# foollh/PicoPose

Hardware: AMD Instinct MI355X
Metric: image-crops/sec (224x224, 162 templates) (higher is better)
Workload: dtype f32 tensors; networks: f32 operands split into 2 f16 terms (22 bits) on f16 MFMA with f32 accumulate; stage-1 contraction: f16 MFMA operands, f32 accumulate, exact f32 re-evaluation of near-ties; PnP f64

## Files before the change

### picopose_amd/csrc/pp_sample.hip

```cpp

#include <hip/hip_runtime.h>
#include <stdint.h>
#include "../../include/picopose_hip.h"
#include "pp_common.h"
#include "pp_corr_dev.h"
#include "pp_crop_dev.h"

namespace {

typedef float f4 __attribute__((ext_vector_type(4)));
typedef _Float16 h8_t __attribute__((ext_vector_type(8)));

__device__ __forceinline__ float resize_blend(float a, float b, float c, float d, float hx, float lx, float hy, float ly, float mul) {
#pragma clang fp contract(off)
    const float top = fmaf(hx, a, lx * b), bot = fmaf(hx, c, lx * d);
    return (hy * top + ly * bot) * mul;
}

__global__ __launch_bounds__(256) void resize_kernel(const float* __restrict__ in, int H, int W, int C,
                                                     int Ho, int Wo, float mul, float* __restrict__ out,
                                                     _Float16* __restrict__ out_hl, int terms) {
    const int b = blockIdx.z, oy = blockIdx.y, tid = threadIdx.x;
    const float sy = Ho > 1 ? (float)(H - 1) / (float)(Ho - 1) : 0.f;
    const float sx = Wo > 1 ? (float)(W - 1) / (float)(Wo - 1) : 0.f;
    const float fy = sy * (float)oy;
    const int y0 = (int)fy, y1 = y0 + (y0 < H - 1 ? 1 : 0);
    const float ly = fy - (float)y0, hy = 1.f - ly;
    const float* ib = in + (size_t)b * H * W * C;
    if (out_hl) {
        _Float16* oh = out_hl + ((size_t)b * Ho + oy) * Wo * terms * C;
        float* of = out ? out + ((size_t)b * Ho + oy) * Wo * C : nullptr;
        const int C8 = C >> 3;
        for (int i = blockIdx.x * 256 + tid; i < Wo * C8; i += gridDim.x * 256) {
            const int ox = i / C8, c = (i - ox * C8) * 8;
            const float fx = sx * (float)ox;
            const int x0 = (int)fx, x1 = x0 + (x0 < W - 1 ? 1 : 0);
            const float lx = fx - (float)x0, hx = 1.f - lx;
            typedef _Float16 h8 __attribute__((ext_vector_type(8)));
            h8 hh, ll;
#pragma unroll
            for (int q = 0; q < 2; ++q) {
                const int cc = c + 4 * q;
                const f4 a = *(const f4*)(ib + ((size_t)y0 * W + x0) * C + cc), bq = *(const f4*)(ib + ((size_t)y0 * W + x1) * C + cc);
                const f4 cq = *(const f4*)(ib + ((size_t)y1 * W + x0) * C + cc), dq = *(const f4*)(ib + ((size_t)y1 * W + x1) * C + cc);
// ... 11 lines not shown
            }
            *(h8*)(oh + ((size_t)ox * C + c) * terms) = hh;
            if (terms == 2) *(h8*)(oh + (size_t)ox * 2 * C + 2 * c + 8) = ll;
        }
        return;
    }
    float* ob = out + ((size_t)b * Ho + oy) * Wo * C;
    if ((C & 3) == 0 && (((uintptr_t)in | (uintptr_t)out) & 15) == 0) {
        const int C4 = C >> 2;
        for (int i = blockIdx.x * 256 + tid; i < Wo * C4; i += gridDim.x * 256) {
            const int ox = i / C4, c = (i - ox * C4) * 4;
            const float fx = sx * (float)ox;
            const int x0 = (int)fx, x1 = x0 + (x0 < W - 1 ? 1 : 0);
            const float lx = fx - (float)x0, hx = 1.f - lx;
            const f4 a = *(const f4*)(ib + ((size_t)y0 * W + x0) * C + c), bq = *(const f4*)(ib + ((size_t)y0 * W + x1) * C + c);
            const f4 cq = *(const f4*)(ib + ((size_t)y1 * W + x0) * C + c), dq = *(const f4*)(ib + ((size_t)y1 * W + x1) * C + c);
            f4 v;
#pragma unroll
            for (int k = 0; k < 4; ++k) v[k] = resize_blend(a[k], bq[k], cq[k], dq[k], hx, lx, hy, ly, mul);
            *(f4*)(ob + (size_t)ox * C + c) = v;
        }
        return;
    }
    for (int i = blockIdx.x * 256 + tid; i < Wo * C; i += gridDim.x * 256) {
        const int ox = i / C, c = i - ox * C;
        const float fx = sx * (float)ox;
        const int x0 = (int)fx, x1 = x0 + (x0 < W - 1 ? 1 : 0);
        const float lx = fx - (float)x0, hx = 1.f - lx;
        ob[i] = resize_blend(ib[((size_t)y0 * W + x0) * C + c], ib[((size_t)y0 * W + x1) * C + c], ib[((size_t)y1 * W + x0) * C + c],
                             ib[((size_t)y1 * W + x1) * C + c], hx, lx, hy, ly, mul);
    }
}

template <bool HL>
__global__ __launch_bounds__(256) void warp_kernel(const float* __restrict__ feat, int feat_batch,
                                                   const float* __restrict__ flow, int H, int W, int C, int ld_flow,
                                                   float* __restrict__ out, int ld_out, int terms) {
    const int b = blockIdx.y, p = blockIdx.x * 4 + (threadIdx.x >> 6), lane = threadIdx.x & 63;
    if (p >= H * W) return;
    const int y = p / W, x = p - y * W;
    const float* fl = flow + ((size_t)b * H * W + p) * ld_flow;
    const float ix = fminf(fmaxf(pp_roundtrip((float)x + fl[0], W), -2.f), (float)W + 1.f);
    const float iy = fminf(fmaxf(pp_roundtrip((float)y + fl[1], H), -2.f), (float)H + 1.f);
    const float x0f = floorf(ix), y0f = floorf(iy);
    const int x0 = (int)x0f, y0 = (int)y0f;
    const float wx1 = ix - x0f, wx0 = (x0f + 1.f) - ix, wy1 = iy - y0f, wy0 = (y0f + 1.f) - iy;
    const float* fb = feat + (size_t)(b % feat_batch) * H * W * C;
    float* o = HL ? nullptr : out + ((size_t)b * H * W + p) * ld_out;
    _Float16* oh = HL ? (_Float16*)out + ((size_t)b * H * W + p) * terms * ld_out : nullptr;
    const bool vx0 = x0 >= 0 && x0 < W, vx1 = x0 + 1 >= 0 && x0 + 1 < W;
    const bool vy0 = y0 >= 0 && y0 < H, vy1 = y0 + 1 >= 0 && y0 + 1 < H;
    typedef unsigned u4w __attribute__((ext_vector_type(4)));
    const unsigned m00 = 0u - (unsigned)(vy0 & vx0), m01 = 0u - (unsigned)(vy0 & vx1), m10 = 0u - (unsigned)(vy1 & vx0),
                   m11 = 0u - (unsigned)(vy1 & vx1);
    const int xa = min(max(x0, 0), W - 1), xb = min(max(x0 + 1, 0), W - 1), ya = min(max(y0, 0), H - 1), yb = min(max(y0 + 1, 0), H - 1);
    auto tap = [&](int yy, int xx, int c, unsigned m) __attribute__((always_inline)) -> f4 {
        const u4w raw = *(const u4w*)(fb + ((size_t)yy * W + xx) * C + c) & m;
        return __builtin_bit_cast(f4, raw);
    };
    for (int c = lane * 4; c < C; c += 256) {
        f4 acc = {0.f, 0.f, 0.f, 0.f};
        acc += tap(ya, xa, c, m00) * (wx0 * wy0);
        acc += tap(ya, xb, c, m01) * (wx1 * wy0);
        acc += tap(yb, xa, c, m10) * (wx0 * wy1);
        acc += tap(yb, xb, c, m11) * (wx1 * wy1);
        if (HL) {
            typedef _Float16 h4w __attribute__((ext_vector_type(4)));
            _Float16 h0, h1, h2, h3, l0, l1, l2, l3;
            pp_split_f16_chk(acc.x, h0, l0);
            pp_split_f16_chk(acc.y, h1, l1);
            pp_split_f16_chk(acc.z, h2, l2);
            pp_split_f16_chk(acc.w, h3, l3);
            if (terms == 2) {
                _Float16* q = oh + pp_hl_col(c, 0);
                *(h4w*)q = h4w{h0, h1, h2, h3};
                *(h4w*)(q + 8) = h4w{l0, l1, l2, l3};
            } else {
                *(h4w*)(oh + c) = h4w{h0, h1, h2, h3};
            }
        } else {
            *(f4*)(o + c) = acc;
        }
    }
}

__global__ __launch_bounds__(256) void avgpool2_kernel(const float* __restrict__ in, int H, int W, int C,
                                                       float* __restrict__ out) {
    const int Ho = H / 2, Wo = W / 2, b = blockIdx.y;
    const size_t n = (size_t)Ho * Wo * C;
    const float* ib = in + (size_t)b * H * W * C;
    float* ob = out + (size_t)b * n;
    for (size_t i = (size_t)blockIdx.x * 256 + threadIdx.x; i < n; i += (size_t)gridDim.x * 256) {
        const int c = (int)(i % C);
        const size_t q = i / C;
        const int ox = (int)(q % Wo), oy = (int)(q / Wo);
        const float* p = ib + ((size_t)(2 * oy) * W + 2 * ox) * C + c;
        ob[i] = ((p[0] + p[C]) + (p[(size_t)W * C] + p[(size_t)W * C + C])) * 0.25f;
    }
}

__global__ __launch_bounds__(256) void avgpool2_hl_kernel(const float* __restrict__ in, int H, int W, int C, float* __restrict__ out,
                                                          _Float16* __restrict__ out_hl) {
    const int Ho = H / 2, Wo = W / 2, b = blockIdx.y, C4 = C >> 2;
    const size_t n4 = (size_t)Ho * Wo * C4;
    const float* ib = in + (size_t)b * H * W * C;
    for (size_t i = (size_t)blockIdx.x * 256 + threadIdx.x; i < n4; i += (size_t)gridDim.x * 256) {
        const int c = (int)(i % C4) * 4;
        const size_t q = i / C4;
        const int ox = (int)(q % Wo), oy = (int)(q / Wo);
        const float* p = ib + ((size_t)(2 * oy) * W + 2 * ox) * C + c;
        const f4 p0 = *(const f4*)p, p1 = *(const f4*)(p + C), p2 = *(const f4*)(p + (size_t)W * C), p3 = *(const f4*)(p + (size_t)W * C + C);
        f4 v;
#pragma unroll
        for (int k = 0; k < 4; ++k) v[k] = ((p0[k] + p1[k]) + (p2[k] + p3[k])) * 0.25f;
        const size_t row = (size_t)b * Ho * Wo + q;
        if (out) *(f4*)(out + row * C + c) = v;
// ... 206 lines not shown
            const int c = i / (np >> 2), q = i - c * (np >> 2);
            *(f4*)&t[c][4 * q] = *(const f4*)(src + (size_t)c * HW + p0 + 4 * q);
        }
    } else {
        for (int i = tid; i < 3 * np; i += 256) {
            const int c = i / np, q = i - c * np;
            t[c][q] = src[(size_t)c * HW + p0 + q];
        }
    }
    __syncthreads();
    h8_t* o = (h8_t*)(out + ((size_t)j * HW + p0) * 8 * terms);
    const _Float16 z = (_Float16)0.f;
    for (int i = tid; i < np * terms; i += 256) {
        const int q = terms == 2 ? i >> 1 : i;
        _Float16 h0, l0, h1, l1, h2, l2;
        if (terms == 1 || (i & 1) == 0) {
            pp_split_f16_chk(t[0][q], h0, l0);
            pp_split_f16_chk(t[1][q], h1, l1);
            pp_split_f16_chk(t[2][q], h2, l2);
            o[i] = h8_t{h0, h1, h2, z, z, z, z, z};
        } else {
            pp_split_f16(t[0][q], h0, l0);
            pp_split_f16(t[1][q], h1, l1);
            pp_split_f16(t[2][q], h2, l2);
            o[i] = h8_t{l0, l1, l2, z, z, z, z, z};
        }
    }
}

}

PP_SAT_SETTER(pp_sat_set_sample)

extern "C" {

int pp_resize_bilinear_nhwc(const float* in, int B, int H, int W, int C, int Ho, int Wo, float mul, float* out,
                            void* stream) {
    if (!in || !out || B <= 0 || H <= 0 || W <= 0 || C <= 0 || Ho <= 0 || Wo <= 0) return PP_EINVAL;
    const bool vec = (C & 3) == 0 && (((uintptr_t)in | (uintptr_t)out) & 15) == 0;
    const int work = vec ? Wo * (C / 4) : Wo * C;
    const int gx = (work + 1023) / 1024;
    hipLaunchKernelGGL(resize_kernel, dim3(gx < 64 ? gx : 64, Ho, B), dim3(256), 0, (hipStream_t)stream, in, H, W,
                       C, Ho, Wo, mul, out, (_Float16*)nullptr, 2);
    return pp_last_launch();
}

int pp_resize_bilinear_nhwc_t(const float* in, int B, int H, int W, int C, int Ho, int Wo, float mul, void* out_hl,
                              int terms, void* stream) {
    if (!in || !out_hl || B <= 0 || H <= 0 || W <= 0 || C <= 0 || C % 8 != 0 || Ho <= 0 || Wo <= 0 ||
        (((uintptr_t)in | (uintptr_t)out_hl) & 15) != 0 || (terms != 1 && terms != 2))
        return PP_EINVAL;
    const int gx = (Wo * (C / 8) + 1023) / 1024;
    hipLaunchKernelGGL(resize_kernel, dim3(gx < 64 ? gx : 64, Ho, B), dim3(256), 0, (hipStream_t)stream, in, H, W,
                       C, Ho, Wo, mul, (float*)nullptr, (_Float16*)out_hl, terms);
    return pp_last_launch();
}

int pp_resize_bilinear_nhwc_dual(const float* in, int B, int H, int W, int C, int Ho, int Wo, float mul, float* out, void* out_hl,
                                 int terms, void* stream) {
    if (!in || !out || !out_hl || B <= 0 || H <= 0 || W <= 0 || C <= 0 || C % 8 != 0 || Ho <= 0 || Wo <= 0 ||
        (((uintptr_t)in | (uintptr_t)out | (uintptr_t)out_hl) & 15) != 0 || (terms != 1 && terms != 2))
        return PP_EINVAL;
    const int gx = (Wo * (C / 8) + 1023) / 1024;
    hipLaunchKernelGGL(resize_kernel, dim3(gx < 64 ? gx : 64, Ho, B), dim3(256), 0, (hipStream_t)stream, in, H, W,
                       C, Ho, Wo, mul, out, (_Float16*)out_hl, terms);
    return pp_last_launch();
}

int pp_resize_bilinear_nhwc_hl(const float* in, int B, int H, int W, int C, int Ho, int Wo, float mul, void* out_hl,
                               void* stream) {
    return pp_resize_bilinear_nhwc_t(in, B, H, W, C, Ho, Wo, mul, out_hl, 2, stream);
}

int pp_warp_nhwc(const float* feat, int feat_batch, const float* flow, int B, int H, int W, int C, int ld_flow,
                 float* out, int ld_out, void* stream) {
    if (!feat || !flow || !out || B <= 0 || H <= 0 || W <= 0 || C <= 0 || C % 4 != 0 || ld_flow < 2 || feat_batch <= 0 ||
        ld_out < C || ld_out % 4 != 0 || ((uintptr_t)out % 16) != 0)
        return PP_EINVAL;
    hipLaunchKernelGGL(warp_kernel<false>, dim3((H * W + 3) / 4, B), dim3(256), 0, (hipStream_t)stream, feat, feat_batch, flow,
                       H, W, C, ld_flow, out, ld_out, 2);
    return pp_last_launch();
}

int pp_warp_nhwc_t(const float* feat, int feat_batch, const float* flow, int B, int H, int W, int C, int ld_flow,
                   void* out_hl, int ld_h, int terms, void* stream) {
    if (!feat || !flow || !out_hl || B <= 0 || H <= 0 || W <= 0 || C <= 0 || C % 8 != 0 || ld_flow < 2 || feat_batch <= 0 ||
        ld_h < C || ld_h % 8 != 0 || ((uintptr_t)out_hl % 16) != 0 || (terms != 1 && terms != 2))
        return PP_EINVAL;
    hipLaunchKernelGGL(warp_kernel<true>, dim3((H * W + 3) / 4, B), dim3(256), 0, (hipStream_t)stream, feat, feat_batch, flow,
                       H, W, C, ld_flow, (float*)out_hl, ld_h, terms);
    return pp_last_launch();
}

int pp_warp_nhwc_hl(const float* feat, int feat_batch, const float* flow, int B, int H, int W, int C, int ld_flow,
                    void* out_hl, int ld_h, void* stream) {
    return pp_warp_nhwc_t(feat, feat_batch, flow, B, H, W, C, ld_flow, out_hl, ld_h, 2, stream);
}

int pp_avgpool2_nhwc(const float* in, int B, int H, int W, int C, float* out, void* stream) {
    if (!in || !out || B <= 0 || H < 2 || W < 2 || C <= 0 || H % 2 != 0 || W % 2 != 0) return PP_EINVAL;
    const size_t n = (size_t)(H / 2) * (W / 2) * C;
    const int gx = (int)((n + 255) / 256 < 1024 ? (n + 255) / 256 : 1024);
    hipLaunchKernelGGL(avgpool2_kernel, dim3(gx, B), dim3(256), 0, (hipStream_t)stream, in, H, W, C, out);
    return pp_last_launch();
}

int pp_avgpool2_hl(const float* in, int B, int H, int W, int C, float* out, void* out_hl, void* stream) {
    if (!in || !out_hl || B <= 0 || H < 2 || W < 2 || C <= 0 || H % 2 != 0 || W % 2 != 0 || C % 8 != 0) return PP_EINVAL;
    if (((uintptr_t)in | (uintptr_t)out | (uintptr_t)out_hl) % 16 != 0) return PP_EINVAL;
    const size_t n = (size_t)(H / 2) * (W / 2) * (C / 4);
    const int gx = (int)((n + 255) / 256 < 1024 ? (n + 255) / 256 : 1024);
    hipLaunchKernelGGL(avgpool2_hl_kernel, dim3(gx, B), dim3(256), 0, (hipStream_t)stream, in, H, W, C, out, (_Float16*)out_hl);
    return pp_last_launch();
}

int pp_conv_narrow_f32(const float* x, int ld_x, int B, int H, int W, int C, const float* weight, const float* bias, int ksize,
                       int n_out, const float* residual, float* out, void* stream) {
    if (!x || !weight || !out || B <= 0 || H <= 0 || C <= 0 || C % 32 != 0 || ld_x < C || ld_x % 4 != 0) return PP_EINVAL;
    if ((W != 16 && W != 32 && W != 64) || H % (256 / W) != 0 || (ksize != 1 && ksize != 3) || (n_out != 1 && n_out != 2)) return PP_EINVAL;
    if (((uintptr_t)x % 16) != 0) return PP_EINVAL;
    const int TH = 256 / W, R = ksize / 2;
    const size_t lds = (size_t)(TH + 2 * R) * (W + 2 * R) * NRW_PITCH;
    const dim3 grid((unsigned)(B * (H / TH)));
// ... 103 lines not shown
```

### picopose_amd/csrc/pp_winograd.hip

```cpp
#include <hip/hip_runtime.h>
#include <stdint.h>
#include "../../include/picopose_hip.h"
#include "pp_common.h"

namespace {

typedef float f4 __attribute__((ext_vector_type(4)));

__device__ __forceinline__ void wino_bt_d_b(const f4 (&d)[4][4], f4 (&u)[4][4]) {
    f4 t[4][4];
#pragma unroll
    for (int c = 0; c < 4; ++c) {
        t[0][c] = d[0][c] - d[2][c];
        t[1][c] = d[1][c] + d[2][c];
        t[2][c] = d[2][c] - d[1][c];
        t[3][c] = d[1][c] - d[3][c];
    }
#pragma unroll
    for (int a = 0; a < 4; ++a) {
        u[a][0] = t[a][0] - t[a][2];
        u[a][1] = t[a][1] + t[a][2];
        u[a][2] = t[a][2] - t[a][1];
        u[a][3] = t[a][1] - t[a][3];
    }
}

__global__ __launch_bounds__(256) void wino_input_kernel(const float* __restrict__ x, int ld_x, long long bstride, int B, int H, int W, int C,
                                                         int relu, float* __restrict__ U) {
    const int c4n = C >> 2;
    const long long P = (long long)B * (H >> 1) * (W >> 1), total = P * c4n;
    for (long long i = (long long)blockIdx.x * 256 + threadIdx.x; i < total; i += (long long)gridDim.x * 256) {
        const long long p = i / c4n;
        const int c = (int)(i - p * c4n) * 4;
        const int tw = W >> 1, th = H >> 1;
        const int b = (int)(p / ((long long)th * tw)), r = (int)(p - (long long)b * th * tw), ty = r / tw, tx = r - ty * tw;
        const int y0 = 2 * ty - 1, x0 = 2 * tx - 1;
// ... 122 lines not shown

__device__ __forceinline__ long long wino_logical_block() {
    const unsigned per = gridDim.x >> 3;
    return (long long)(blockIdx.x & 7) * per + (blockIdx.x >> 3);
}

#define PP_W4_BT(d0, d1, d2, d3, d4, d5, t0, t1, t2, t3, t4, t5)          \
    {                                                                     \
        const f4 a_ = d4 - 4.f * d2, b_ = d3 - 4.f * d1;                  \
        const f4 c_ = d4 - d2, e_ = 2.f * (d3 - d1);                      \
        t0 = 4.f * d0 - 5.f * d2 + d4;                                    \
        t1 = a_ + b_;                                                     \
        t2 = a_ - b_;                                                     \
        t3 = c_ + e_;                                                     \
        t4 = c_ - e_;                                                     \
        t5 = 4.f * d1 - 5.f * d3 + d5;                                    \
    }

__device__ __forceinline__ void wino_split4(f4 v, hf4& hi, hf4& lo, float& top) {
    top = fmaxf(fmaxf(top, fabsf(v[0])), fabsf(v[1]));
    top = fmaxf(fmaxf(top, fabsf(v[2])), fabsf(v[3]));
#pragma unroll
    for (int e = 0; e < 4; ++e) {
        const _Float16 h = (_Float16)v[e];
        hi[e] = h;
        lo[e] = (_Float16)(v[e] - (float)h);
    }
}

__device__ __forceinline__ void wino_note_sat(bool clamp, unsigned* sat) {
    if (sat && __builtin_amdgcn_ballot_w64(clamp) != 0ull && (threadIdx.x & 63) == 0) atomicOr(sat, 1u);
}

typedef unsigned int wu4 __attribute__((ext_vector_type(4)));
__device__ __forceinline__ unsigned wino_swap(unsigned v) { return (unsigned)__builtin_amdgcn_mov_dpp((int)v, 0xB1, 0xF, 0xF, true); }
__device__ __forceinline__ float wino_h2f(unsigned w, int hi16) { return (float)__builtin_bit_cast(_Float16, (unsigned short)(hi16 ? w >> 16 : w & 0xFFFFu)); }

__device__ __forceinline__ f4 wino_pair_unpack(wu4 q, int par) {
    const unsigned k0 = par ? q[2] : q[0], k1 = par ? q[3] : q[1];
    const unsigned r0 = wino_swap(par ? q[0] : q[2]), r1 = wino_swap(par ? q[1] : q[3]);
    return f4{wino_h2f(k0, 0) + wino_h2f(r0, 0), wino_h2f(k0, 1) + wino_h2f(r0, 1), wino_h2f(k1, 0) + wino_h2f(r1, 0), wino_h2f(k1, 1) + wino_h2f(r1, 1)};
}

__device__ __forceinline__ wu4 wino_pair_pack(int par, hf4 hi, hf4 lo) {
    const unsigned H0 = __builtin_bit_cast(unsigned, __builtin_shufflevector(hi, hi, 0, 1)), H1 = __builtin_bit_cast(unsigned, __builtin_shufflevector(hi, hi, 2, 3));
    const unsigned L0 = __builtin_bit_cast(unsigned, __builtin_shufflevector(lo, lo, 0, 1)), L1 = __builtin_bit_cast(unsigned, __builtin_shufflevector(lo, lo, 2, 3));
    const unsigned r0 = wino_swap(par ? H0 : L0), r1 = wino_swap(par ? H1 : L1);
    return wu4{par ? r0 : H0, par ? r1 : H1, par ? L0 : r0, par ? L1 : r1};
}

__device__ __forceinline__ __amdgpu_buffer_rsrc_t wino_block_rsrc(const void* base, int xi, unsigned long long block_bytes) {
    return __builtin_amdgcn_make_buffer_rsrc((void*)((const char*)base + (unsigned long long)xi * block_bytes), 0, (int)(unsigned)block_bytes, 0x00020000);
}

__device__ __forceinline__ void wino_pair_store(_Float16* grp, int par, hf4 hi, hf4 lo) {
    const unsigned H0 = __builtin_bit_cast(unsigned, __builtin_shufflevector(hi, hi, 0, 1)), H1 = __builtin_bit_cast(unsigned, __builtin_shufflevector(hi, hi, 2, 3));
    const unsigned L0 = __builtin_bit_cast(unsigned, __builtin_shufflevector(lo, lo, 0, 1)), L1 = __builtin_bit_cast(unsigned, __builtin_shufflevector(lo, lo, 2, 3));
    const unsigned r0 = wino_swap(par ? H0 : L0), r1 = wino_swap(par ? H1 : L1);
    const wu4 w = {par ? r0 : H0, par ? r1 : H1, par ? L0 : r0, par ? L1 : r1};
    *(wu4*)(grp + par * 8) = w;
}

template <bool RELU>
__global__ __launch_bounds__(256, 2) void wino4_input_kernel(const _Float16* __restrict__ x, unsigned x_bytes, int ld_x, long long bstride, int B, int H,
                                                             int W, int C, _Float16* __restrict__ U, long long Pp, unsigned* sat) {
    const int c4n = C >> 2;
    const int tw = W >> 2, th = H >> 2;
    const long long P = (long long)B * th * tw, total = P * c4n;
    const long long i = wino_logical_block() * 256 + threadIdx.x;
    if (i >= total) return;
    const long long p = i / c4n;
    const int c = (int)(i - p * c4n) * 4;
    const int b = (int)(p / ((long long)th * tw)), r = (int)(p - (long long)b * th * tw), ty = r / tw, tx = r - ty * tw;
    const int y0 = 4 * ty - 1, x0 = 4 * tx - 1;
    const int gcol = (c >> 3) << 4;
    const int par = (c >> 2) & 1;
    const unsigned pix = (unsigned)ld_x * 4u;
    const unsigned back = (unsigned)(W + 1) * pix;
    const __amdgpu_buffer_rsrc_t R = __builtin_amdgcn_make_buffer_rsrc((void*)((const char*)x - back), 0, (int)(x_bytes + back), 0x00020000);
    const unsigned v00 = (unsigned)((b * bstride * 2 + gcol + par * 8) * 2) + (unsigned)((y0 + 1) * W + x0 + 1) * pix;
    bool rok[6], cok[6];
#pragma unroll
    for (int k = 0; k < 6; ++k) {
        rok[k] = (unsigned)(y0 + k) < (unsigned)H;
        cok[k] = (unsigned)(x0 + k) < (unsigned)W;
    }
    wu4 q[6][6];
#pragma unroll
    for (int dx = 0; dx < 6; ++dx)
#pragma unroll
        for (int dy = 0; dy < 6; ++dy)
            q[dy][dx] = __builtin_amdgcn_raw_buffer_load_b128(R, (rok[dy] && cok[dx]) ? v00 : 0xFFFFFFFFu, (dy * W + dx) * (int)pix, 0);
    f4 t[6][6];
#pragma unroll
    for (int dx = 0; dx < 6; ++dx) {
        f4 d[6];
#pragma unroll
        for (int dy = 0; dy < 6; ++dy) {
            f4 v = wino_pair_unpack(q[dy][dx], par);
            if (RELU) {
#pragma unroll
                for (int e = 0; e < 4; ++e) v[e] = fmaxf(v[e], 0.f);
            }
            d[dy] = v;
        }
        PP_W4_BT(d[0], d[1], d[2], d[3], d[4], d[5], t[0][dx], t[1][dx], t[2][dx], t[3][dx], t[4][dx], t[5][dx])
    }
    float top = 0.f;
    const unsigned long long blk = (unsigned long long)Pp * C * 4;
    const unsigned uoff = (unsigned)((p * 2 * C + gcol + par * 8) * 2);
#pragma unroll
    for (int a = 0; a < 6; ++a) {
        f4 u[6];
        PP_W4_BT(t[a][0], t[a][1], t[a][2], t[a][3], t[a][4], t[a][5], u[0], u[1], u[2], u[3], u[4], u[5])
#pragma unroll
        for (int bb = 0; bb < 6; ++bb) {
            hf4 hi, lo;
            wino_split4(u[bb] * (1.f / 64.f), hi, lo, top);
            __builtin_amdgcn_raw_buffer_store_b128(wino_pair_pack(par, hi, lo), wino_block_rsrc(U, 6 * a + bb, blk), uoff, 0, PP_WINO_ST_AUX);
        }
    }
    wino_note_sat(!(top < 65504.f), sat);
}

__global__ __launch_bounds__(256) void wino4_weight_kernel(const float* __restrict__ w, int Cout, int Cin, int ldw, float* __restrict__ V) {
    const long long total = (long long)Cout * Cin;
    const long long i = (long long)blockIdx.x * 256 + threadIdx.x;
    if (i >= total) return;
    const int co = (int)(i / Cin), ci = (int)(i - (long long)co * Cin);
    float g[3][3], t[6][3];
#pragma unroll
    for (int ky = 0; ky < 3; ++ky)
#pragma unroll
        for (int kx = 0; kx < 3; ++kx) g[ky][kx] = w[(long long)co * ldw + (ky * 3 + kx) * Cin + ci];
    auto g6 = [](float g0, float g1, float g2, float (&o)[6]) {
        o[0] = 0.25f * g0;
        o[1] = (-1.f / 6.f) * ((g0 + g2) + g1);
        o[2] = (-1.f / 6.f) * ((g0 + g2) - g1);
        o[3] = (1.f / 24.f) * g0 + (1.f / 12.f) * g1 + (1.f / 6.f) * g2;
        o[4] = (1.f / 24.f) * g0 - (1.f / 12.f) * g1 + (1.f / 6.f) * g2;
        o[5] = g2;
    };
#pragma unroll
    for (int kx = 0; kx < 3; ++kx) {
        float o[6];
        g6(g[0][kx], g[1][kx], g[2][kx], o);
#pragma unroll
        for (int a = 0; a < 6; ++a) t[a][kx] = o[a];
    }
#pragma unroll
    for (int a = 0; a < 6; ++a) {
        float o[6];
// ... 32 lines not shown
        f4 y[6];
#pragma unroll
        for (int a = 0; a < 6; ++a) y[a] = __builtin_bit_cast(f4, __builtin_amdgcn_raw_buffer_load_b128(wino_block_rsrc(Y, 6 * a + bb, blk), yoff, 0, PP_WINO_LD_AUX));
        PP_W4_AT(y[0], y[1], y[2], y[3], y[4], y[5], z[0][bb], z[1][bb], z[2][bb], z[3][bb])
    }
    const f4 bv = bias ? *(const f4*)(bias + c) : f4{0.f, 0.f, 0.f, 0.f};
    const float slope = act == PP_ACT_RELU ? 0.f : (act == PP_ACT_LEAKY01 ? 0.1f : 1.f);
    const float hfloor = c_relu ? 0.f : -INFINITY;
    const int gcol = (c >> 3) << 4, par = (c >> 2) & 1;
    float top = 0.f;
#pragma unroll
    for (int oy = 0; oy < 4; ++oy) {
        f4 o[4];
        PP_W4_AT(z[oy][0], z[oy][1], z[oy][2], z[oy][3], z[oy][4], z[oy][5], o[0], o[1], o[2], o[3])
#pragma unroll
        for (int ox = 0; ox < 4; ++ox) {
            const long long row = ((long long)b * H + 4 * ty + oy) * W + 4 * tx + ox;
            f4 v = o[ox] + bv;
#pragma unroll
            for (int e = 0; e < 4; ++e) v[e] = fmaxf(v[e], v[e] * slope);
            if (out) {
                f4 w = v;
                if (residual) w += *(const f4*)(residual + row * ldc + c);
                if (residual2) w += *(const f4*)(residual2 + row * ldc + c);
                *(f4*)(out + row * ldc + c) = w;
                v = w;
            }
            if (out_hl) {
                hf4 hi, lo;
                f4 x4;
#pragma unroll
                for (int e = 0; e < 4; ++e) x4[e] = fmaxf(v[e] * PP_A_SCALE, hfloor);
                wino_split4(x4, hi, lo, top);
                wino_pair_store(out_hl + row * 2 * ld_h + gcol, par, hi, lo);
            }
        }
    }
    wino_note_sat(!(top < 65504.f), sat);
}

constexpr int CHN_PX = 36;
__device__ __forceinline__ int wino_opaque(int xi) {
    int k;
    asm volatile("s_mov_b32 %0, %1" : "=s"(k) : "s"(xi));
    return k;
}

template <int W, int NB>
__global__ __launch_bounds__((1 + NB) * ((W / 4) * 8 < 64 ? 64 : (W / 4) * 8)) void wino4_chain_kernel(const float* __restrict__ Y, int H, int C, const float* __restrict__ bias,
                                                                       int act, int c_relu, _Float16* __restrict__ U, long long Pp, int ldy, unsigned* sat) {
    constexpr int TW = W / 4, NI = TW * 8;
    constexpr int GS = NI < 64 ? 64 : NI;
    constexpr int SLOT = 4 * W * CHN_PX;
    extern __shared__ __attribute__((aligned(16))) float chs[];
    const int th = H >> 2, nsl = C >> 5;
    const int b = blockIdx.x / nsl, cs = blockIdx.x - b * nsl;
    const int half = NB == 2 ? __builtin_amdgcn_readfirstlane((int)threadIdx.x / GS) : (int)threadIdx.x / GS;
    const int it = (int)threadIdx.x - half * GS, tx = it >> 3, q = it & 7;
    const bool live = NI >= GS || it < NI;
    const int c = cs * 32 + 4 * q;
    const unsigned long long blk = (unsigned long long)Pp * C * 4, blky = (unsigned long long)Pp * ldy * 4;
    const f4 bv = bias ? *(const f4*)(bias + c) : f4{0.f, 0.f, 0.f, 0.f};
    const float slope = act == PP_ACT_RELU ? 0.f : (act == PP_ACT_LEAKY01 ? 0.1f : 1.f);
    const int gcol = (c >> 3) << 4, par = q & 1;
    const float hfloor = c_relu ? 0.f : -INFINITY;
    float top = 0.f;
    for (int r = 0; r < th + 2; ++r) {
// ... 36 lines not shown
#pragma unroll
            for (int dx = 0; dx < 6; ++dx) {
                f4 d[6];
                const int px = 4 * tx - 1 + dx;
#pragma unroll
                for (int dy = 0; dy < 6; ++dy) {
                    const int g = 4 * R - 1 + dy;
                    const int gc = min(max(g, 0), H - 1), pc = min(max(px, 0), W - 1);
                    f4 v = *(const f4*)(chs + ((gc >> 2) & 3) * SLOT + ((gc & 3) * W + pc) * CHN_PX + 4 * q);
                    if (!(g >= 0 && g < H && px >= 0 && px < W)) v = f4{0.f, 0.f, 0.f, 0.f};
                    d[dy] = v;
                }
                PP_W4_BT(d[0], d[1], d[2], d[3], d[4], d[5], t[0][dx], t[1][dx], t[2][dx], t[3][dx], t[4][dx], t[5][dx])
            }
            const long long p = ((long long)b * th + R) * TW + tx;
            const unsigned uoff = (unsigned)((p * 2 * C + gcol + par * 8) * 2);
#pragma unroll
            for (int ai = 0; ai < RPG; ++ai) {
                f4 u[6];
                if constexpr (NB == 2) {
                    f4 t0 = t[ai][0], t1 = t[ai][1], t2 = t[ai][2], t3 = t[ai][3], t4 = t[ai][4], t5 = t[ai][5];
                    if (a0) {
                        t0 = t[3 + ai][0], t1 = t[3 + ai][1], t2 = t[3 + ai][2];
                        t3 = t[3 + ai][3], t4 = t[3 + ai][4], t5 = t[3 + ai][5];
                    }
                    PP_W4_BT(t0, t1, t2, t3, t4, t5, u[0], u[1], u[2], u[3], u[4], u[5])
                } else {
                    PP_W4_BT(t[ai][0], t[ai][1], t[ai][2], t[ai][3], t[ai][4], t[ai][5], u[0], u[1], u[2], u[3], u[4], u[5])
                }
#pragma unroll
                for (int bb = 0; bb < 6; ++bb) {
                    hf4 hi, lo;
                    wino_split4(u[bb] * (1.f / 64.f), hi, lo, top);
                    __builtin_amdgcn_raw_buffer_store_b128(wino_pair_pack(par, hi, lo), wino_block_rsrc(U, wino_opaque(6 * (a0 + ai) + bb), blk), uoff, 0, PP_WINO_ST_AUX);
                }
            }
        }
        __syncthreads();
    }
    wino_note_sat(!(top < 65504.f), sat);
}

template <int W>
__global__ __launch_bounds__(2 * (W / 2) * 8, 4) void wino2_chain_kernel(const float* __restrict__ Y, int H, int C, long long P, const float* __restrict__ bias,
                                                                       int act, int relu_next, float* __restrict__ U) {
    constexpr int TW = W / 2, NI = TW * 8;
    constexpr int SLOT = 2 * W * CHN_PX;
    extern __shared__ __attribute__((aligned(16))) float chs[];
    const int th = H >> 1, nsl = C >> 5;
    const int b = blockIdx.x / nsl, cs = blockIdx.x - b * nsl;
    const int half = threadIdx.x / NI, it = threadIdx.x - half * NI, tx = it >> 3, q = it & 7;
    const int c = cs * 32 + 4 * q;
    const f4 bv = bias ? *(const f4*)(bias + c) : f4{0.f, 0.f, 0.f, 0.f};
    for (int r = 0; r < th + 2; ++r) {
        if (half == 0 && r < th) {
            const long long p = ((long long)b * th + r) * TW + tx;
            f4 y[4][4];
#pragma unroll
            for (int a = 0; a < 4; ++a)
#pragma unroll
                for (int bb = 0; bb < 4; ++bb) y[a][bb] = *(const f4*)(Y + ((long long)(4 * a + bb) * P + p) * C + c);
            float* slot = chs + (r & 3) * SLOT;
#pragma unroll
            for (int oy = 0; oy < 2; ++oy)
#pragma unroll
                for (int ox = 0; ox < 2; ++ox) {
                    f4 col[4], o;
// ... 184 lines not shown
```

Measured before the change: 583.6.

## Add paired-store resize and multi-pixel warp kernels for split-f16 operand output

Adds a new resize kernel in which each wave handles runs of output pixels. It issues all four tap loads for several pixels before blending, and writes hi/lo f16 terms with a DPP lane-pair swap, so each lane emits one full 16-byte store instead of two 8-byte ones. Adds a warp (grid-sample) kernel that computes tap offsets and weights once per pixel, broadcasts them with readlane, and processes two pixels per wave. It also remaps block order across hypotheses and tiles. The pair pack/unpack helpers move into a shared header, and environment variables can restore the old kernels. The saturation check is now a wave-level flag, and the paths use 32-bit offsets guarded by size checks.

```diff
diff --git a/picopose_amd/csrc/pp_pair_dev.h b/picopose_amd/csrc/pp_pair_dev.h
--- /dev/null
+++ b/picopose_amd/csrc/pp_pair_dev.h
@@ -0,0 +1,32 @@
+#ifndef PP_PAIR_DEV_H
+#define PP_PAIR_DEV_H
+#include <hip/hip_runtime.h>
+
+namespace {
+
+typedef float pair_f4 __attribute__((ext_vector_type(4)));
+typedef _Float16 pair_h4 __attribute__((ext_vector_type(4)));
+typedef unsigned int pair_u4 __attribute__((ext_vector_type(4)));
+
+__device__ __forceinline__ unsigned pair_swap(unsigned v) { return (unsigned)__builtin_amdgcn_mov_dpp((int)v, 0xB1, 0xF, 0xF, true); }
+__device__ __forceinline__ float pair_h2f(unsigned w, int hi16) { return (float)__builtin_bit_cast(_Float16, (unsigned short)(hi16 ? w >> 16 : w & 0xFFFFu)); }
+
+__device__ __forceinline__ pair_f4 pair_unpack(pair_u4 q, int par) {
+    const unsigned k0 = par ? q[2] : q[0], k1 = par ? q[3] : q[1];
+    const unsigned r0 = pair_swap(par ? q[0] : q[2]), r1 = pair_swap(par ? q[1] : q[3]);
+    return pair_f4{pair_h2f(k0, 0) + pair_h2f(r0, 0), pair_h2f(k0, 1) + pair_h2f(r0, 1), pair_h2f(k1, 0) + pair_h2f(r1, 0), pair_h2f(k1, 1) + pair_h2f(r1, 1)};
+}
+
+__device__ __forceinline__ pair_u4 pair_pack(int par, pair_h4 hi, pair_h4 lo) {
+    const unsigned H0 = __builtin_bit_cast(unsigned, __builtin_shufflevector(hi, hi, 0, 1)), H1 = __builtin_bit_cast(unsigned, __builtin_shufflevector(hi, hi, 2, 3));
+    const unsigned L0 = __builtin_bit_cast(unsigned, __builtin_shufflevector(lo, lo, 0, 1)), L1 = __builtin_bit_cast(unsigned, __builtin_shufflevector(lo, lo, 2, 3));
+    const unsigned r0 = pair_swap(par ? H0 : L0), r1 = pair_swap(par ? H1 : L1);
+    return pair_u4{par ? r0 : H0, par ? r1 : H1, par ? L0 : r0, par ? L1 : r1};
+}
+
+__device__ __forceinline__ void pair_store(_Float16* grp, int par, pair_h4 hi, pair_h4 lo) {
+    *(pair_u4*)(grp + par * 8) = pair_pack(par, hi, lo);
+}
+
+}
+#endif
diff --git a/picopose_amd/csrc/pp_sample.hip b/picopose_amd/csrc/pp_sample.hip
--- a/picopose_amd/csrc/pp_sample.hip
+++ b/picopose_amd/csrc/pp_sample.hip
@@ -1,15 +1,19 @@
 
 #include <hip/hip_runtime.h>
 #include <stdint.h>
+#include <stdlib.h>
 #include "../../include/picopose_hip.h"
 #include "pp_common.h"
 #include "pp_corr_dev.h"
 #include "pp_crop_dev.h"
+#include "pp_pair_dev.h"
 
 namespace {
 
 typedef float f4 __attribute__((ext_vector_type(4)));
 typedef _Float16 h8_t __attribute__((ext_vector_type(8)));
+typedef _Float16 h4w __attribute__((ext_vector_type(4)));
+typedef unsigned u4w __attribute__((ext_vector_type(4)));
 
 __device__ __forceinline__ float resize_blend(float a, float b, float c, float d, float hx, float lx, float hy, float ly, float mul) {
 #pragma clang fp contract(off)
@@ -87,6 +91,99 @@
     }
 }
 
+__device__ __forceinline__ void split4_f16(f4 v, h4w& hi, h4w& lo, bool& bad) {
+#pragma unroll
+    for (int k = 0; k < 4; ++k) {
+        bad |= !(fabsf(v[k]) * PP_A_SCALE < 65504.f);
+        _Float16 h, l;
+        pp_split_f16(v[k], h, l);
+        hi[k] = h;
+        lo[k] = l;
+    }
+}
+__device__ __forceinline__ u4w load16(const float* base, unsigned off) { return *(const u4w*)((const char*)base + off); }
+
+constexpr int RESIZE_RUN = 4;
+__global__ __launch_bounds__(256) void resize_pair_kernel(const float* __restrict__ in, int H, int W, int C, int Ho, int Wo, float mul,
+                                                          float* __restrict__ out, _Float16* __restrict__ out_hl, int terms, int lp_log2) {
+    const int b = blockIdx.z, oy = blockIdx.y, lane = threadIdx.x & 63, par = lane & 1;
+    const float sy = Ho > 1 ? (float)(H - 1) / (float)(Ho - 1) : 0.f;
+    const float sx = Wo > 1 ? (float)(W - 1) / (float)(Wo - 1) : 0.f;
+    const float fy = sy * (float)oy;
+    const int y0 = (int)fy, y1 = y0 + (y0 < H - 1 ? 1 : 0);
+    const float ly = fy - (float)y0, hy = 1.f - ly;
+    const float* r0 = in + ((size_t)b * H + y0) * W * C;
+    const float* r1 = in + ((size_t)b * H + y1) * W * C;
+    _Float16* oh = out_hl + ((size_t)b * Ho + oy) * Wo * terms * C;
+    float* of = out ? out + ((size_t)b * Ho + oy) * Wo * C : nullptr;
+    const int ppw = 64 >> lp_log2;
+    const int ox0 = ((blockIdx.x * 4 + __builtin_amdgcn_readfirstlane(threadIdx.x >> 6)) * RESIZE_RUN) * ppw + (lane >> lp_log2);
+    int ox[RESIZE_RUN];
+    unsigned t0[RESIZE_RUN], t1[RESIZE_RUN];
+    float lx[RESIZE_RUN];
+#pragma unroll
+    for (int r = 0; r < RESIZE_RUN; ++r) {
+        ox[r] = ox0 + r * ppw;
+        const float fx = sx * (float)min(ox[r], Wo - 1);
+        const int x0 = (int)fx, x1 = x0 + (x0 < W - 1 ? 1 : 0);
+        lx[r] = fx - (float)x0;
+        t0[r] = (unsigned)(x0 * C) * 4u, t1[r] = (unsigned)(x1 * C) * 4u;
+    }
+    bool bad = false;
+    for (int c = (lane & ((1 << lp_log2) - 1)) * 4; c < C; c += 4 << lp_log2) {
+        u4w a[RESIZE_RUN], bq[RESIZE_RUN], cq[RESIZE_RUN], dq[RESIZE_RUN];
+#pragma unroll
+        for (int r = 0; r < RESIZE_RUN; ++r) {
+            a[r] = load16(r0, t0[r] + 4u * c), bq[r] = load16(r0, t1[r] + 4u * c);
+            cq[r] = load16(r1, t0[r] + 4u * c), dq[r] = load16(r1, t1[r] + 4u * c);
+        }
+#pragma unroll
+        for (int r = 0; r < RESIZE_RUN; ++r) {
+            if (ox[r] >= Wo) continue;
+            const float hx = 1.f - lx[r];
+            const f4 fa = __builtin_bit_cast(f4, a[r]), fb = __builtin_bit_cast(f4, bq[r]), fc = __builtin_bit_cast(f4, cq[r]), fd = __builtin_bit_cast(f4, dq[r]);
+            f4 v;
+#pragma unroll
+            for (int k = 0; k < 4; ++k) v[k] = resize_blend(fa[k], fb[k], fc[k], fd[k], hx, lx[r], hy, ly, mul);
+            h4w hi, lo;
+            split4_f16(v, hi, lo, bad);
+            const unsigned e = (unsigned)(ox[r] * C + c);
+            if (of) *(f4*)((char*)of + 4u * e) = v;
+            if (terms == 2) pair_store((_Float16*)((char*)oh + 4u * (e & ~7u)), par, hi, lo);
+            else *(h4w*)((char*)oh + 2u * e) = hi;
+        }
+    }
+    pp_sat_flag(bad);
+}
+
+
+struct WarpTaps {
+    int xa, xb, ya, yb;
+    unsigned m00, m01, m10, m11;
+    float wx0, wx1, wy0, wy1;
+};
+__device__ __forceinline__ WarpTaps warp_taps(const float* __restrict__ fl, int x, int y, int H, int W) {
+    const float ix = fminf(fmaxf(pp_roundtrip((float)x + fl[0], W), -2.f), (float)W + 1.f);
+    const float iy = fminf(fmaxf(pp_roundtrip((float)y + fl[1], H), -2.f), (float)H + 1.f);
+    const float x0f = floorf(ix), y0f = floorf(iy);
+    const int x0 = (int)x0f, y0 = (int)y0f;
+    WarpTaps t;
+    t.wx1 = ix - x0f, t.wx0 = (x0f + 1.f) - ix, t.wy1 = iy - y0f, t.wy0 = (y0f + 1.f) - iy;
+    const bool vx0 = x0 >= 0 && x0 < W, vx1 = x0 + 1 >= 0 && x0 + 1 < W;
+    const bool vy0 = y0 >= 0 && y0 < H, vy1 = y0 + 1 >= 0 && y0 + 1 < H;
+    t.m00 = 0u - (unsigned)(vy0 & vx0), t.m01 = 0u - (unsigned)(vy0 & vx1), t.m10 = 0u - (unsigned)(vy1 & vx0), t.m11 = 0u - (unsigned)(vy1 & vx1);
+    t.xa = min(max(x0, 0), W - 1), t.xb = min(max(x0 + 1, 0), W - 1), t.ya = min(max(y0, 0), H - 1), t.yb = min(max(y0 + 1, 0), H - 1);
+    return t;
+}
+__device__ __forceinline__ f4 warp_masked(u4w raw, unsigned m) { return __builtin_bit_cast(f4, raw & m); }
+__device__ __forceinline__ f4 warp_blend(const WarpTaps& t, f4 v00, f4 v01, f4 v10, f4 v11) {
+    const float w00 = t.wx0 * t.wy0, w01 = t.wx1 * t.wy0, w10 = t.wx0 * t.wy1, w11 = t.wx1 * t.wy1;
+    f4 acc;
+#pragma unroll
+    for (int k = 0; k < 4; ++k) acc[k] = fmaf(v11[k], w11, fmaf(v10[k], w10, fmaf(v01[k], w01, fmaf(v00[k], w00, 0.f))));
+    return acc;
+}
+
 template <bool HL>
 __global__ __launch_bounds__(256) void warp_kernel(const float* __restrict__ feat, int feat_batch,
                                                    const float* __restrict__ flow, int H, int W, int C, int ld_flow,
@@ -94,33 +191,16 @@
     const int b = blockIdx.y, p = blockIdx.x * 4 + (threadIdx.x >> 6), lane = threadIdx.x & 63;
     if (p >= H * W) return;
     const int y = p / W, x = p - y * W;
-    const float* fl = flow + ((size_t)b * H * W + p) * ld_flow;
-    const float ix = fminf(fmaxf(pp_roundtrip((float)x + fl[0], W), -2.f), (float)W + 1.f);
-    const float iy = fminf(fmaxf(pp_roundtrip((float)y + fl[1], H), -2.f), (float)H + 1.f);
-    const float x0f = floorf(ix), y0f = floorf(iy);
-    const int x0 = (int)x0f, y0 = (int)y0f;
-    const float wx1 = ix - x0f, wx0 = (x0f + 1.f) - ix, wy1 = iy - y0f, wy0 = (y0f + 1.f) - iy;
+    const WarpTaps t = warp_taps(flow + ((size_t)b * H * W + p) * ld_flow, x, y, H, W);
     const float* fb = feat + (size_t)(b % feat_batch) * H * W * C;
     float* o = HL ? nullptr : out + ((size_t)b * H * W + p) * ld_out;
     _Float16* oh = HL ? (_Float16*)out + ((size_t)b * H * W + p) * terms * ld_out : nullptr;
-    const bool vx0 = x0 >= 0 && x0 < W, vx1 = x0 + 1 >= 0 && x0 + 1 < W;
-    const bool vy0 = y0 >= 0 && y0 < H, vy1 = y0 + 1 >= 0 && y0 + 1 < H;
-    typedef unsigned u4w __attribute__((ext_vector_type(4)));
-    const unsigned m00 = 0u - (unsigned)(vy0 & vx0), m01 = 0u - (unsigned)(vy0 & vx1), m10 = 0u - (unsigned)(vy1 & vx0),
-                   m11 = 0u - (unsigned)(vy1 & vx1);
-    const int xa = min(max(x0, 0), W - 1), xb = min(max(x0 + 1, 0), W - 1), ya = min(max(y0, 0), H - 1), yb = min(max(y0 + 1, 0), H - 1);
     auto tap = [&](int yy, int xx, int c, unsigned m) __attribute__((always_inline)) -> f4 {
-        const u4w raw = *(const u4w*)(fb + ((size_t)yy * W + xx) * C + c) & m;
-        return __builtin_bit_cast(f4, raw);
+        return warp_masked(*(const u4w*)(fb + ((size_t)yy * W + xx) * C + c), m);
     };
     for (int c = lane * 4; c < C; c += 256) {
-        f4 acc = {0.f, 0.f, 0.f, 0.f};
-        acc += tap(ya, xa, c, m00) * (wx0 * wy0);
-        acc += tap(ya, xb, c, m01) * (wx1 * wy0);
-        acc += tap(yb, xa, c, m10) * (wx0 * wy1);
-        acc += tap(yb, xb, c, m11) * (wx1 * wy1);
+        const f4 acc = warp_blend(t, tap(t.ya, t.xa, c, t.m00), tap(t.ya, t.xb, c, t.m01), tap(t.yb, t.xa, c, t.m10), tap(t.yb, t.xb, c, t.m11));
         if (HL) {
-            typedef _Float16 h4w __attribute__((ext_vector_type(4)));
             _Float16 h0, h1, h2, h3, l0, l1, l2, l3;
             pp_split_f16_chk(acc.x, h0, l0);
             pp_split_f16_chk(acc.y, h1, l1);
@@ -137,6 +217,67 @@
             *(f4*)(o + c) = acc;
         }
     }
+}
+
+constexpr int WARP_RUN = 2;
+__device__ __forceinline__ float readlane_f(float v, int l) { return __builtin_bit_cast(float, __builtin_amdgcn_readlane(__builtin_bit_cast(int, v), l)); }
+__global__ __launch_bounds__(256) void warp_run_kernel(const float* __restrict__ feat, int feat_batch, const float* __restrict__ flow, int H,
+                                                       int W, int C, int ld_flow, _Float16* __restrict__ out, int ld_out, int terms, int hyps,
+                                                       int nimg, int tiles) {
+    const int lane = threadIdx.x & 63, par = lane & 1, HW = H * W;
+    const unsigned per = gridDim.x >> 3;
+    const unsigned item = (blockIdx.x & 7) * per + (blockIdx.x >> 3);
+    const int hyp = item % hyps, tile = (item / hyps) % tiles, img = item / hyps / tiles;
+    if (img >= nimg) return;
+    const int b = hyp * nimg + img;
+    const int p0 = (tile * 4 + __builtin_amdgcn_readfirstlane(threadIdx.x >> 6)) * WARP_RUN;
+    if (p0 >= HW) return;
+    const float* fb = feat + (size_t)(b % feat_batch) * HW * C;
+    int o[WARP_RUN][4];
+    unsigned m[WARP_RUN][4];
+    float w[WARP_RUN][4];
+    {
+        const int pl = min(p0 + min(lane, WARP_RUN - 1), HW - 1), y = pl / W, x = pl - y * W;
+        const WarpTaps t = warp_taps(flow + ((size_t)b * HW + pl) * ld_flow, x, y, H, W);
+        const int o00 = (t.ya * W + t.xa) * C, o01 = (t.ya * W + t.xb) * C, o10 = (t.yb * W + t.xa) * C, o11 = (t.yb * W + t.xb) * C;
+        const float w00 = t.wx0 * t.wy0, w01 = t.wx1 * t.wy0, w10 = t.wx0 * t.wy1, w11 = t.wx1 * t.wy1;
+        const int mbits = (int)((t.m00 & 1u) | (t.m01 & 2u) | (t.m10 & 4u) | (t.m11 & 8u));
+#pragma unroll
+        for (int r = 0; r < WARP_RUN; ++r) {
+            o[r][0] = __builtin_amdgcn_readlane(o00, r), o[r][1] = __builtin_amdgcn_readlane(o01, r);
+            o[r][2] = __builtin_amdgcn_readlane(o10, r), o[r][3] = __builtin_amdgcn_readlane(o11, r);
+            w[r][0] = readlane_f(w00, r), w[r][1] = readlane_f(w01, r), w[r][2] = readlane_f(w10, r), w[r][3] = readlane_f(w11, r);
+            const unsigned mb = (unsigned)__builtin_amdgcn_readlane(mbits, r);
+#pragma unroll
+            for (int q = 0; q < 4; ++q) m[r][q] = 0u - ((mb >> q) & 1u);
+        }
+    }
+    bool bad = false;
+    for (int c = lane * 4; c < C; c += 256) {
+        u4w raw[WARP_RUN][4];
+#pragma unroll
+        for (int r = 0; r < WARP_RUN; ++r)
+#pragma unroll
+            for (int q = 0; q < 4; ++q) raw[r][q] = load16(fb, 4u * (unsigned)(o[r][q] + c));
+#pragma unroll
+        for (int r = 0; r < WARP_RUN; ++r) {
+            if (p0 + r >= HW) break;
+            f4 acc;
+#pragma unroll
+            for (int k = 0; k < 4; ++k) {
+                float s = fmaf(__builtin_bit_cast(float, raw[r][0][k] & m[r][0]), w[r][0], 0.f);
+                s = fmaf(__builtin_bit_cast(float, raw[r][1][k] & m[r][1]), w[r][1], s);
+                s = fmaf(__builtin_bit_cast(float, raw[r][2][k] & m[r][2]), w[r][2], s);
+                acc[k] = fmaf(__builtin_bit_cast(float, raw[r][3][k] & m[r][3]), w[r][3], s);
+            }
+            h4w hi, lo;
+            split4_f16(acc, hi, lo, bad);
+            _Float16* oh = out + ((size_t)b * HW + p0 + r) * terms * ld_out;
+            if (terms == 2) pair_store((_Float16*)((char*)oh + 4u * (unsigned)(c & ~7)), par, hi, lo);
+            else *(h4w*)((char*)oh + 2u * (unsigned)c) = hi;
+        }
+    }
+    pp_sat_flag(bad);
 }
 
 __global__ __launch_bounds__(256) void avgpool2_kernel(const float* __restrict__ in, int H, int W, int C,
@@ -409,6 +550,22 @@
 
 PP_SAT_SETTER(pp_sat_set_sample)
 
+static int launch_resize_operand(const float* in, int B, int H, int W, int C, int Ho, int Wo, float mul, float* out, _Float16* out_hl, int terms,
+                                 hipStream_t st) {
+    const char* re = getenv("PP_RESIZE_PAIRS");
+    if ((re && re[0] == '0') || (long long)(W > Wo ? W : Wo) * C > 0x7FFFFFFFLL / 4) {
+        const int gx = (Wo * (C / 8) + 1023) / 1024;
+        hipLaunchKernelGGL(resize_kernel, dim3(gx < 64 ? gx : 64, Ho, B), dim3(256), 0, st, in, H, W, C, Ho, Wo, mul, out, out_hl, terms);
+        return pp_last_launch();
+    }
+    int lp_log2 = 1;
+    while (lp_log2 < 6 && (4 << lp_log2) < C) ++lp_log2;
+    const int per_block = 4 * RESIZE_RUN * (64 >> lp_log2);
+    hipLaunchKernelGGL(resize_pair_kernel, dim3((Wo + per_block - 1) / per_block, Ho, B), dim3(256), 0, st, in, H, W, C, Ho, Wo, mul, out, out_hl,
+                       terms, lp_log2);
+    return pp_last_launch();
+}
+
 extern "C" {
 
 int pp_resize_bilinear_nhwc(const float* in, int B, int H, int W, int C, int Ho, int Wo, float mul, float* out,
@@ -427,10 +584,7 @@
     if (!in || !out_hl || B <= 0 || H <= 0 || W <= 0 || C <= 0 || C % 8 != 0 || Ho <= 0 || Wo <= 0 ||
         (((uintptr_t)in | (uintptr_t)out_hl) & 15) != 0 || (terms != 1 && terms != 2))
         return PP_EINVAL;
-    const int gx = (Wo * (C / 8) + 1023) / 1024;
-    hipLaunchKernelGGL(resize_kernel, dim3(gx < 64 ? gx : 64, Ho, B), dim3(256), 0, (hipStream_t)stream, in, H, W,
-                       C, Ho, Wo, mul, (float*)nullptr, (_Float16*)out_hl, terms);
-    return pp_last_launch();
+    return launch_resize_operand(in, B, H, W, C, Ho, Wo, mul, nullptr, (_Float16*)out_hl, terms, (hipStream_t)stream);
 }
 
 int pp_resize_bilinear_nhwc_dual(const float* in, int B, int H, int W, int C, int Ho, int Wo, float mul, float* out, void* out_hl,
@@ -438,10 +592,7 @@
     if (!in || !out || !out_hl || B <= 0 || H <= 0 || W <= 0 || C <= 0 || C % 8 != 0 || Ho <= 0 || Wo <= 0 ||
         (((uintptr_t)in | (uintptr_t)out | (uintptr_t)out_hl) & 15) != 0 || (terms != 1 && terms != 2))
         return PP_EINVAL;
-    const int gx = (Wo * (C / 8) + 1023) / 1024;
-    hipLaunchKernelGGL(resize_kernel, dim3(gx < 64 ? gx : 64, Ho, B), dim3(256), 0, (hipStream_t)stream, in, H, W,
-                       C, Ho, Wo, mul, out, (_Float16*)out_hl, terms);
-    return pp_last_launch();
+    return launch_resize_operand(in, B, H, W, C, Ho, Wo, mul, out, (_Float16*)out_hl, terms, (hipStream_t)stream);
 }
 
 int pp_resize_bilinear_nhwc_hl(const float* in, int B, int H, int W, int C, int Ho, int Wo, float mul, void* out_hl,
@@ -464,8 +615,17 @@
     if (!feat || !flow || !out_hl || B <= 0 || H <= 0 || W <= 0 || C <= 0 || C % 8 != 0 || ld_flow < 2 || feat_batch <= 0 ||
         ld_h < C || ld_h % 8 != 0 || ((uintptr_t)out_hl % 16) != 0 || (terms != 1 && terms != 2))
         return PP_EINVAL;
-    hipLaunchKernelGGL(warp_kernel<true>, dim3((H * W + 3) / 4, B), dim3(256), 0, (hipStream_t)stream, feat, feat_batch, flow,
-                       H, W, C, ld_flow, (float*)out_hl, ld_h, terms);
+    const char* re = getenv("PP_WARP_RUN");
+    if ((re && re[0] == '0') || (long long)H * W * C > 0x7FFFFFFFLL / 4)
+        hipLaunchKernelGGL(warp_kernel<true>, dim3((H * W + 3) / 4, B), dim3(256), 0, (hipStream_t)stream, feat, feat_batch, flow,
+                           H, W, C, ld_flow, (float*)out_hl, ld_h, terms);
+    else {
+        const int hyps = B % feat_batch == 0 ? B / feat_batch : 1, tiles = (H * W + 4 * WARP_RUN - 1) / (4 * WARP_RUN);
+        const long long blocks = ((long long)tiles * B + 7) / 8 * 8;
+        if (blocks > 0x7FFFFFFFLL) return PP_EINVAL;
+        hipLaunchKernelGGL(warp_run_kernel, dim3((unsigned)blocks), dim3(256), 0, (hipStream_t)stream, feat, feat_batch, flow, H, W, C, ld_flow,
+                           (_Float16*)out_hl, ld_h, terms, hyps, B / hyps, tiles);
+    }
     return pp_last_launch();
 }
 
diff --git a/picopose_amd/csrc/pp_winograd.hip b/picopose_amd/csrc/pp_winograd.hip
--- a/picopose_amd/csrc/pp_winograd.hip
+++ b/picopose_amd/csrc/pp_winograd.hip
@@ -2,6 +2,7 @@
 #include <stdint.h>
 #include "../../include/picopose_hip.h"
 #include "pp_common.h"
+#include "pp_pair_dev.h"
 
 namespace {
 
@@ -190,33 +191,8 @@
     if (sat && __builtin_amdgcn_ballot_w64(clamp) != 0ull && (threadIdx.x & 63) == 0) atomicOr(sat, 1u);
 }
 
-typedef unsigned int wu4 __attribute__((ext_vector_type(4)));
-__device__ __forceinline__ unsigned wino_swap(unsigned v) { return (unsigned)__builtin_amdgcn_mov_dpp((int)v, 0xB1, 0xF, 0xF, true); }
-__device__ __forceinline__ float wino_h2f(unsigned w, int hi16) { return (float)__builtin_bit_cast(_Float16, (unsigned short)(hi16 ? w >> 16 : w & 0xFFFFu)); }
-
-__device__ __forceinline__ f4 wino_pair_unpack(wu4 q, int par) {
-    const unsigned k0 = par ? q[2] : q[0], k1 = par ? q[3] : q[1];
-    const unsigned r0 = wino_swap(par ? q[0] : q[2]), r1 = wino_swap(par ? q[1] : q[3]);
-    return f4{wino_h2f(k0, 0) + wino_h2f(r0, 0), wino_h2f(k0, 1) + wino_h2f(r0, 1), wino_h2f(k1, 0) + wino_h2f(r1, 0), wino_h2f(k1, 1) + wino_h2f(r1, 1)};
-}
-
-__device__ __forceinline__ wu4 wino_pair_pack(int par, hf4 hi, hf4 lo) {
-    const unsigned H0 = __builtin_bit_cast(unsigned, __builtin_shufflevector(hi, hi, 0, 1)), H1 = __builtin_bit_cast(unsigned, __builtin_shufflevector(hi, hi, 2, 3));
-    const unsigned L0 = __builtin_bit_cast(unsigned, __builtin_shufflevector(lo, lo, 0, 1)), L1 = __builtin_bit_cast(unsigned, __builtin_shufflevector(lo, lo, 2, 3));
-    const unsigned r0 = wino_swap(par ? H0 : L0), r1 = wino_swap(par ? H1 : L1);
-    return wu4{par ? r0 : H0, par ? r1 : H1, par ? L0 : r0, par ? L1 : r1};
-}
-
 __device__ __forceinline__ __amdgpu_buffer_rsrc_t wino_block_rsrc(const void* base, int xi, unsigned long long block_bytes) {
     return __builtin_amdgcn_make_buffer_rsrc((void*)((const char*)base + (unsigned long long)xi * block_bytes), 0, (int)(unsigned)block_bytes, 0x00020000);
-}
-
-__device__ __forceinline__ void wino_pair_store(_Float16* grp, int par, hf4 hi, hf4 lo) {
-    const unsigned H0 = __builtin_bit_cast(unsigned, __builtin_shufflevector(hi, hi, 0, 1)), H1 = __builtin_bit_cast(unsigned, __builtin_shufflevector(hi, hi, 2, 3));
-    const unsigned L0 = __builtin_bit_cast(unsigned, __builtin_shufflevector(lo, lo, 0, 1)), L1 = __builtin_bit_cast(unsigned, __builtin_shufflevector(lo, lo, 2, 3));
-    const unsigned r0 = wino_swap(par ? H0 : L0), r1 = wino_swap(par ? H1 : L1);
-    const wu4 w = {par ? r0 : H0, par ? r1 : H1, par ? L0 : r0, par ? L1 : r1};
-    *(wu4*)(grp + par * 8) = w;
 }
 
 template <bool RELU>
@@ -243,7 +219,7 @@
         rok[k] = (unsigned)(y0 + k) < (unsigned)H;
         cok[k] = (unsigned)(x0 + k) < (unsigned)W;
     }
-    wu4 q[6][6];
+    pair_u4 q[6][6];
 #pragma unroll
     for (int dx = 0; dx < 6; ++dx)
 #pragma unroll
@@ -255,7 +231,7 @@
         f4 d[6];
 #pragma unroll
         for (int dy = 0; dy < 6; ++dy) {
-            f4 v = wino_pair_unpack(q[dy][dx], par);
+            f4 v = pair_unpack(q[dy][dx], par);
             if (RELU) {
 #pragma unroll
                 for (int e = 0; e < 4; ++e) v[e] = fmaxf(v[e], 0.f);
@@ -275,7 +251,7 @@
         for (int bb = 0; bb < 6; ++bb) {
             hf4 hi, lo;
             wino_split4(u[bb] * (1.f / 64.f), hi, lo, top);
-            __builtin_amdgcn_raw_buffer_store_b128(wino_pair_pack(par, hi, lo), wino_block_rsrc(U, 6 * a + bb, blk), uoff, 0, PP_WINO_ST_AUX);
+            __builtin_amdgcn_raw_buffer_store_b128(pair_pack(par, hi, lo), wino_block_rsrc(U, 6 * a + bb, blk), uoff, 0, PP_WINO_ST_AUX);
         }
     }
     wino_note_sat(!(top < 65504.f), sat);
@@ -374,7 +350,7 @@
 #pragma unroll
                 for (int e = 0; e < 4; ++e) x4[e] = fmaxf(v[e] * PP_A_SCALE, hfloor);
                 wino_split4(x4, hi, lo, top);
-                wino_pair_store(out_hl + row * 2 * ld_h + gcol, par, hi, lo);
+                pair_store(out_hl + row * 2 * ld_h + gcol, par, hi, lo);
             }
         }
     }
@@ -477,7 +453,7 @@
                 for (int bb = 0; bb < 6; ++bb) {
                     hf4 hi, lo;
                     wino_split4(u[bb] * (1.f / 64.f), hi, lo, top);
-                    __builtin_amdgcn_raw_buffer_store_b128(wino_pair_pack(par, hi, lo), wino_block_rsrc(U, wino_opaque(6 * (a0 + ai) + bb), blk), uoff, 0, PP_WINO_ST_AUX);
+                    __builtin_amdgcn_raw_buffer_store_b128(pair_pack(par, hi, lo), wino_block_rsrc(U, wino_opaque(6 * (a0 + ai) + bb), blk), uoff, 0, PP_WINO_ST_AUX);
                 }
             }
         }
```

Result: no change. 585.9, median of 6 (+0.4%).
